# ZhangT-tech/MoCA-Video

Hardware: AMD Instinct MI355X
Metric: denoising UNet-steps/sec @16x320x512 fp16 (higher is better)
Workload: dtype f16

## Files before the change

include/moca_hip.h:

```cpp
#ifndef MOCA_HIP_H
#define MOCA_HIP_H

#include <stdint.h>

#ifdef __cplusplus
extern "C" {
#endif

#define MOCA_OK            0
#define MOCA_E_BADARG     -1
#define MOCA_E_LAUNCH     -2
#define MOCA_E_NODEVICE   -3
#define MOCA_E_GRAPH      -4

#define MOCA_A_LINEAR   0
#define MOCA_A_CONV3X3  1
#define MOCA_A_TCONV3   2

#define MOCA_EP_GEGLU   1
#define MOCA_EP_OUT_F32 2
#define MOCA_FORCE_SMALL_TILE 4
#define MOCA_EP_COLSUM 16
#define MOCA_EP_LN     32
#define MOCA_EP_GELU    8
// ... 44 lines not shown
    float       tattn_scale;
    const void* prefetch;
    int32_t     up_phase;
    int32_t     reserved4_;
    const void* a2;
    int32_t     lda2;
    int32_t     k1;
    int32_t     gstat_cpg;
    int32_t     gstat_coff;
    int32_t     wgroup_rows;
    int32_t     wgroup_stride;
} moca_gemm_params;

int moca_gemm_f16(const moca_gemm_params* p, void* stream);
int moca_gemm_colsum_rows(const moca_gemm_params* p);
int moca_gemm_ln_ok(const moca_gemm_params* p);
int moca_gemm_rowsum_cols(const moca_gemm_params* p);
int moca_gemm_lnfold_ok(const moca_gemm_params* p);
int moca_gemm_tattn_ok(const moca_gemm_params* p);
int moca_gemm_wgroup_ok(const moca_gemm_params* p);
int moca_gemm_cat_ok(const moca_gemm_params* p);
#define MOCA_ROUTE_SMALL64   1
#define MOCA_ROUTE_SMALL128  2
#define MOCA_ROUTE_GLDS128   3
#define MOCA_ROUTE_GLDS160   4
#define MOCA_ROUTE_G4        5
#define MOCA_ROUTE_W80       6
#define MOCA_ROUTE_W80W      7
#define MOCA_ROUTE_SQ256     8
#define MOCA_ROUTE_G4P       9
#define MOCA_ROUTE_SQP       10
#define MOCA_ROUTE_TATTN     11
#define MOCA_ROUTE_WS        12
int moca_gemm_route(const moca_gemm_params* p);
int moca_gemm_splitk_groupnorm_ok(const moca_gemm_params* p, int32_t HW, int32_t frames_per_stat);
int moca_gemm_splitk_groupnorm_f16(const moca_gemm_params* p, void* y, const float* gamma, const float* beta, int32_t HW,
                                   int32_t frames_per_stat, float eps, int32_t silu, int32_t write_x, void* stream);
int64_t moca_gemm_splitk_ws_bytes(int32_t M, int32_t N, int32_t splits);

int moca_groupnorm_nhwc_f16(const void* x, void* y, const float* gamma, const float* beta,
                            int32_t F, int32_t HW, int32_t C, int32_t frames_per_stat,
                            float eps, int32_t silu, float* ws, void* stream);
int64_t moca_groupnorm_ws_bytes(int32_t F, int32_t HW, int32_t C);
int moca_groupnorm_colsum_f16(const void* x, void* y, const float* gamma, const float* beta, const float* colsum,
                              int32_t tile_rows, int32_t F, int32_t HW, int32_t C, int32_t frames_per_stat,
                              float eps, int32_t silu, float* ws, void* stream);

int moca_groupnorm_fold_weights_f16(const void* w, const float* bias, const float* gamma, const float* beta, const int64_t* gstat,
                                    void* wg, float* bg, int32_t n_sg, int32_t N, int32_t K, int32_t ldw, int64_t count, float eps,
                                    void* stream);

int moca_groupnorm_gstat_f16(const void* x, void* y, const float* gamma, const float* beta, const int64_t* gstat,
                             int32_t F, int32_t HW, int32_t C, int32_t frames_per_stat,
                             float eps, int32_t silu, void* stream);
int moca_concat_channels_gstat_f16(const void* a, const void* b, void* out, int32_t F, int32_t HW, int32_t C1, int32_t C2,
                                   int32_t frames_per_stat, int64_t* gstat, void* stream);
int moca_groupnorm_gstat_cat_f16(const void* a, const void* b, void* y, const float* gamma, const float* beta,
                                 const int64_t* gstat_cat, const int64_t* gstat_b, int32_t Fb, int32_t F, int32_t HW, int32_t C1,
                                 int32_t C2, int32_t frames_per_stat, float eps, int32_t silu, void* stream);
int moca_gstat_accum_f16(const void* x, int32_t F, int32_t HW, int32_t C, int32_t frames_per_stat, int32_t cpg, int32_t coff,
                         int64_t* gstat, void* stream);
int moca_memset_zero(void* ptr, int64_t bytes, void* stream);

int moca_layernorm_f16(const void* x, void* y, const float* gamma, const float* beta,
                       int32_t M, int32_t C, float eps, void* stream);

// ... 117 lines not shown
int moca_base_ddim_step_f32(moca_fifo_state* state, float* x, const float* eps_c, const float* eps_u, const float* noise,
                            float* pred_x0, const float* coef, int32_t S, float cfg_scale, int32_t use_scale, int64_t n, void* stream);
int moca_mask_frame_sums_f32(const float* mask, float* sums, int32_t frames, int32_t HW, void* stream);

int moca_freq_mix_3d_f32(const float* x, const float* noise, const float* lpf, float* out,
                         int32_t C, int32_t T, int32_t H, int32_t W, float* ws, void* stream);
int64_t moca_freq_mix_ws_bytes(int32_t C, int32_t T, int32_t H, int32_t W);
int moca_freq_filter_f32(float* lpf, int32_t T, int32_t H, int32_t W, int32_t type, int32_t n,
                         double d_s, double d_t, void* stream);

int moca_graph_begin(void* stream);
int moca_graph_end(void* stream, void** graph_exec_out);
int moca_graph_launch(void* graph_exec, void* stream);
int moca_graph_destroy(void* graph_exec);
int moca_stream_create(void** stream_out);
int moca_stream_destroy(void* stream);
int moca_stream_sync(void* stream);
int moca_event_create(void** ev_out);
int moca_event_record(void* ev, void* stream);
int moca_event_elapsed_ms(void* ev_start, void* ev_stop, float* ms_out);
int moca_event_destroy(void* ev);

#define MOCA_TUNE_GEMM_W80   0
#define MOCA_TUNE_GEMM_G4    1
#define MOCA_TUNE_GEMM_SQ256 2
#define MOCA_TUNE_GEMM_WIDE  3
#define MOCA_TUNE_GN_SLAB    4
#define MOCA_TUNE_GEMM_G4P   5
#define MOCA_TUNE_GEMM_MF32  6
#define MOCA_TUNE_GEMM_SQP   7
#define MOCA_TUNE_SQP_WALK   8
#define MOCA_TUNE_SLAB_F16   9
#define MOCA_TUNE_GEMM_WS    10
#define MOCA_TUNE_COUNT      11
int moca_set_tuning(int32_t knob, int32_t value);
int moca_debug_clock_sampler(void* buf, int32_t blocks, int32_t nsamples, const int32_t* stop, void* stream);

int moca_device_info(char* name, int32_t len, int32_t* cu_count);
const char* moca_version(void);

#ifdef __cplusplus
}
#endif
#endif
```

moca_video_amd/csrc/gemm.hip:

```cpp
#include "gemm_launch.h"

namespace {

template <int BN, int AMODE>
__global__ __launch_bounds__(256, 2) void gemm_f16_kernel(const moca_gemm_params p) {
    constexpr int NT = BN / 64;
    constexpr int B_SLOTS = BN / 32;
    constexpr int A_BYTES = BM * ROW_BYTES;
    constexpr int B_BYTES = BN * ROW_BYTES;

    extern __shared__ __attribute__((aligned(16))) char smem[];
    char* sA = smem;
    char* sB = smem + 2 * A_BYTES;

    const int tid = threadIdx.x, lane = tid & 63, wave = tid >> 6;
    const int wave_m = wave >> 1, wave_n = wave & 1;

    const int tiles_m = (p.M + BM - 1) / BM;
    const int tiles_n = p.N / BN;
    const int nblk = tiles_m * tiles_n * p.splits;
    int logical;
    remap_block<BN>(nblk, logical);
    const int split = logical % p.splits;
    const int tile = logical / p.splits;
// ... 389 lines not shown
            const int c0 = ccol[i] - g * cpg;
            half8v r;
#pragma unroll
            for (int j = 0; j < 8; ++j) {
                float a = (float)v[i][j] * s_sc[c0 + j] + s_sh[c0 + j];
                if (silu) a = moca_silu(a);
                r[j] = (half_t)a;
            }
            *reinterpret_cast<half8v*>(y + (int64_t)mrow[i] * N + ccol[i]) = r;
        }
}

template <int BN, int AMODE>
int launch_gemm(const moca_gemm_params& p, hipStream_t st) {
    const int tiles_m = (p.M + BM - 1) / BM, tiles_n = p.N / BN;
    const int nblk = tiles_m * tiles_n * p.splits;
    constexpr int lds_pipe = 2 * (BM + BN) * ROW_BYTES;
    constexpr int lds_epi = BM * BN * 4;
    constexpr int lds = lds_pipe > lds_epi ? lds_pipe : lds_epi;
    if (!dyn_lds_once<&gemm_f16_kernel<BN, AMODE>>(lds)) return MOCA_E_LAUNCH;
    hipLaunchKernelGGL((gemm_f16_kernel<BN, AMODE>), dim3(nblk), dim3(256), lds, st, p);
    MOCA_CHECK_LAUNCH();
    return MOCA_OK;
}
int launch_gemm_small(int bn, const moca_gemm_params& p, hipStream_t st) {
    if (bn == 128) return with_gather(p, [&](auto am, auto) { return launch_gemm<128, decltype(am)::value>(p, st); });
    return with_gather(p, [&](auto am, auto) { return launch_gemm<64, decltype(am)::value>(p, st); });
}

enum Route : int {
    R_NONE = 0,
    R_SMALL64 = MOCA_ROUTE_SMALL64, R_SMALL128 = MOCA_ROUTE_SMALL128, R_GLDS128 = MOCA_ROUTE_GLDS128, R_GLDS160 = MOCA_ROUTE_GLDS160,
    R_G4 = MOCA_ROUTE_G4, R_W80 = MOCA_ROUTE_W80, R_W80W = MOCA_ROUTE_W80W, R_SQ256 = MOCA_ROUTE_SQ256, R_G4P = MOCA_ROUTE_G4P,
    R_SQP = MOCA_ROUTE_SQP, R_TATTN = MOCA_ROUTE_TATTN, R_WS = MOCA_ROUTE_WS,
};

void normalise_splits(moca_gemm_params& p) {
    if (p.splits < 1) p.splits = 1;
    if (p.splits > (p.K + BK - 1) / BK) p.splits = (p.K + BK - 1) / BK;
    if (p.splits > 1) {
        const int nkt = (p.K + BK - 1) / BK, kts = (nkt + p.splits - 1) / p.splits;
        p.splits = (nkt + kts - 1) / kts;
    }
}

inline int64_t a_span_bytes(const moca_gemm_params& p) {
    if (p.a_mode == MOCA_A_LINEAR) return ((int64_t)p.M * p.lda + 64) * 2;
    if (p.a_mode == MOCA_A_CONV3X3) return ((int64_t)(p.M / (p.outH * p.outW)) * p.inH * p.inW * p.C + 64) * 2;
    return ((int64_t)p.M * p.C + 64) * 2;
}
inline bool buffer_addressable(const moca_gemm_params& p) {
    if (p.a2 && ((int64_t)p.M * p.lda2 + 64) * 2 >= (1ll << 31)) return false;
    return a_span_bytes(p) < (1ll << 31) && (int64_t)p.N * p.ldw * 2 < (1ll << 31);
}

bool persistent_ok(const moca_gemm_params& p, int BN, int blocks) {
    if (p.a_mode != MOCA_A_LINEAR || p.splits != 1 || p.N % BN || p.K % 64 || !buffer_addressable(p)) return false;
    if (p.flags & ~(MOCA_EP_GEGLU | MOCA_EP_LNFOLD)) return false;
    if ((p.flags & MOCA_EP_GEGLU) && (p.residual || p.rowadd)) return false;
    return ((p.M + 255) / 256) * (p.N / BN) >= blocks;
}

Route route_of(const moca_gemm_params& p) {
    if (p.flags & MOCA_EP_TATTN) return R_TATTN;
    const int ws_mode = moca_tuning_get(MOCA_TUNE_GEMM_WS);
    if (ws_mode && moca_gemm_ws_ok(p) && (ws_mode == 2 || p.residual || p.M >= (1 << 17))) return R_WS;
    if (!p.a2 && p.wgroup_rows <= 0) {
        const int sqp_mode = moca_tuning_get(MOCA_TUNE_GEMM_SQP), g4p_mode = moca_tuning_get(MOCA_TUNE_GEMM_G4P);
        if (sqp_mode && persistent_ok(p, 256, SQP_BLOCKS) && (sqp_mode == 2 || (p.flags & MOCA_EP_GEGLU))) return R_SQP;
        if (g4p_mode && persistent_ok(p, 128, G4P_BLOCKS) && (g4p_mode == 2 || (p.flags & MOCA_EP_GEGLU))) return R_G4P;
    }
    const int w80_mode = moca_tuning_get(MOCA_TUNE_GEMM_W80);
    const int tiles320 = ((p.M + 319) / 320) * (p.N / 160);
    if (w80_mode && p.N % 160 == 0 && !(p.flags & (MOCA_EP_GEGLU | MOCA_EP_OUT_F32 | MOCA_FORCE_SMALL_TILE)) && p.M > 160 &&
        (tiles320 * p.splits >= 200 || w80_mode == 2) && fast_gather(p) && buffer_addressable(p)) {
        if (p.flags & MOCA_EP_LN) return R_W80W;
        const int wide_mode = moca_tuning_get(MOCA_TUNE_GEMM_WIDE);
        if (wide_mode == 0 || p.N % 320) return R_W80;
        return (p.a_mode == MOCA_A_LINEAR || wide_mode == 2) ? R_W80W : R_W80;
    }
    const int g4_mode = moca_tuning_get(MOCA_TUNE_GEMM_G4);
    const bool use_g4 = !(p.flags & MOCA_EP_OUT_F32) &&
                        (g4_mode == 2 || (g4_mode == 1 && (p.flags & MOCA_EP_GEGLU) && p.K <= 640 && p.M < (1 << 17)));
    const int sq256_mode = moca_tuning_get(MOCA_TUNE_GEMM_SQ256);
    if (sq256_mode && p.a_mode == MOCA_A_LINEAR && p.N % 256 == 0 && p.N >= 2560 && p.M >= 512 && fast_gather(p) && buffer_addressable(p) &&
        !(p.flags & (MOCA_EP_OUT_F32 | MOCA_FORCE_SMALL_TILE)) && ((p.M + 255) / 256) * (p.N / 256) * p.splits >= 200 &&
        (sq256_mode == 2 || !use_g4)) return R_SQ256;
    const int big_bn = (p.N % 128 == 0) ? 128 : (p.N % 160 == 0 ? 160 : 0);
    if (big_bn != 0 && p.M > 128 && !(p.flags & MOCA_FORCE_SMALL_TILE)) {
        if (big_bn == 128) return use_g4 ? R_G4 : R_GLDS128;
        return R_GLDS160;
    }
    return p.N % 128 == 0 ? R_SMALL128 : R_SMALL64;
}

constexpr int CAN_SPLITK = 1 << 16, CAN_A2 = 1 << 17, CAN_WGROUP = 1 << 18, CAN_UP_PHASE = 1 << 19;
constexpr int EP_STATS = MOCA_EP_COLSUM | MOCA_EP_GSTAT;
struct RouteInfo { int tm, tn, can; };
RouteInfo route_info(Route r) {
    constexpr int GLDS = MOCA_EP_GEGLU | MOCA_EP_OUT_F32 | EP_STATS | MOCA_EP_ROWSUM | MOCA_EP_LNFOLD | CAN_SPLITK | CAN_UP_PHASE;
    constexpr int W80 = EP_STATS | MOCA_EP_ROWSUM | MOCA_EP_LNFOLD | CAN_SPLITK | CAN_UP_PHASE | CAN_A2 | CAN_WGROUP;
    switch (r) {
        case R_SMALL64: return {BM, 64, MOCA_EP_OUT_F32 | MOCA_EP_GELU | CAN_SPLITK};
        case R_SMALL128: return {BM, 128, MOCA_EP_GEGLU | MOCA_EP_OUT_F32 | MOCA_EP_GELU | CAN_SPLITK};
        case R_GLDS128: return {256, 128, GLDS};
        case R_GLDS160: return {256, 160, GLDS};
        case R_G4: return {256, 128, MOCA_EP_GEGLU | MOCA_EP_LNFOLD | CAN_SPLITK | CAN_UP_PHASE};
        case R_W80: return {320, 160, W80};
        case R_W80W: return {160, 320, W80 | MOCA_EP_LN};
        case R_SQ256: return {256, 256, MOCA_EP_GEGLU | MOCA_EP_LNFOLD | CAN_SPLITK};
        case R_G4P: return {256, 128, MOCA_EP_GEGLU | MOCA_EP_LNFOLD};
        case R_SQP: return {256, 256, MOCA_EP_GEGLU | MOCA_EP_LNFOLD};
        case R_TATTN: return {320, 192, MOCA_EP_TATTN | MOCA_EP_LNFOLD};
        case R_WS: return {32, 80, MOCA_EP_ROWSUM | MOCA_EP_GSTAT | CAN_WGROUP};
        case R_NONE: break;
    }
    return {0, 0, 0};
}

bool route_can(Route r, const moca_gemm_params& p) {
    const RouteInfo ri = route_info(r);
    const int f = p.flags & ~(MOCA_FORCE_SMALL_TILE | MOCA_EP_SLABS);
    const int wants = f | (p.splits > 1 ? CAN_SPLITK : 0) | (p.a2 ? CAN_A2 : 0) | (p.wgroup_rows ? CAN_WGROUP : 0) | (p.up_phase ? CAN_UP_PHASE : 0);
    if (r == R_NONE || (wants & ~ri.can) || p.wgroup_rows < 0) return false;
    if (r == R_WS) return true;
    const bool linear1 = p.a_mode == MOCA_A_LINEAR && p.splits == 1;
    if (r == R_TATTN) {
        if (!linear1 || !fast_gather(p) || !buffer_addressable(p) || p.residual || p.rowadd || (p.flags & MOCA_FORCE_SMALL_TILE)) return false;
        if (p.N % 192 || p.T != 16 || p.HW <= 0 || p.HW % 20 || p.M % (16 * p.HW)) return false;
        if (p.ldo % 4 || p.ldo < p.N / 3) return false;
        return p.tattn_causal == 0 || (p.tattn_causal == 1 && p.tattn_scale > 0.f);
    }
    if ((f & EP_STATS) && (p.splits != 1 || (f & (MOCA_EP_GEGLU | MOCA_EP_OUT_F32)))) return false;
    if ((f & MOCA_EP_ROWSUM) && (p.splits != 1 || (f & (MOCA_EP_GEGLU | MOCA_EP_OUT_F32 | EP_STATS | MOCA_EP_LN | MOCA_EP_GELU)))) return false;
    if ((f & MOCA_EP_LN) && !(linear1 && p.N == 320 && !(f & EP_STATS))) return false;
    if ((f & MOCA_EP_LNFOLD) && !(linear1 && !(f & (MOCA_EP_OUT_F32 | EP_STATS | MOCA_EP_LN | MOCA_EP_ROWSUM | MOCA_EP_GELU)) &&
                                  !((r == R_GLDS128 || r == R_GLDS160) && (f & MOCA_EP_GEGLU)))) return false;
    if ((f & MOCA_EP_GELU) && (f & MOCA_EP_GEGLU)) return false;
    if (p.a2) {
        if (!linear1 || (f & ~(EP_STATS | MOCA_EP_ROWSUM))) return false;
        if (p.k1 <= 0 || p.k1 >= p.K || p.k1 % 64 || (p.K - p.k1) % 64 || p.lda % 8 || p.lda2 % 8 || p.lda < p.k1 || p.lda2 < p.K - p.k1) return false;
    }
    if (p.wgroup_rows) {
        if (!linear1 || p.a2 || p.wgroup_stride < p.N * p.ldw || (f & ~(EP_STATS | MOCA_EP_ROWSUM | MOCA_EP_LN))) return false;
        if (p.M % p.wgroup_rows || p.wgroup_rows % ri.tm) return false;
        if ((int64_t)(p.M / p.wgroup_rows) * p.wgroup_stride * 2 >= (1ll << 31)) return false;
    }
    if (p.up_phase && (p.splits != 1 || p.M <= 160 || !fast_gather(p) || p.residual || p.rowadd || (f & ~MOCA_EP_GSTAT) ||
                       (p.N % 128 && p.N % 160))) return false;
    return true;
}

Route checked_route(const moca_gemm_params& p) {
    const Route r = route_of(p);
    return route_can(r, p) ? r : R_NONE;
}

Route query_route(const moca_gemm_params* pp, int flag, moca_gemm_params& p) {
// ... 44 lines not shown
            if (p.up && (p.stride != 1 || p.outH != 2 * p.inH || p.outW != 2 * p.inW)) return R_NONE;
            if (!p.up && p.stride == 1 && (p.outH != p.inH || p.outW != p.inW)) return R_NONE;
            if (p.stride == 2 && (p.outH != (p.inH - 1) / 2 + 1 || p.outW != (p.inW - 1) / 2 + 1)) return R_NONE;
            if (p.M % (p.outH * p.outW)) return R_NONE;
            break;
        case MOCA_A_TCONV3:
            if (p.C % 8 || p.K != 3 * p.C || p.T <= 0 || p.HW <= 0 || p.M % (p.T * p.HW)) return R_NONE;
            break;
        default:
            return R_NONE;
    }
    if (p.a2 && p.a_mode != MOCA_A_LINEAR) return R_NONE;
    if (p.gstat_cpg < 0 || p.gstat_coff < 0 || ((p.gstat_cpg || p.gstat_coff) && !(p.flags & MOCA_EP_GSTAT))) return R_NONE;
    if (p.tattn_causal && !(p.flags & MOCA_EP_TATTN)) return R_NONE;
    const Route r = checked_route(p);
    if (r == R_NONE) return R_NONE;
    if ((p.flags & MOCA_EP_COLSUM) && !p.colsum) return R_NONE;
    if ((p.flags & MOCA_EP_LN) && !(p.ln_gamma && p.ln_beta && p.ln_out && p.ld_ln % 8 == 0)) return R_NONE;
    if ((p.flags & MOCA_EP_ROWSUM) && !p.rowsum) return R_NONE;
    if ((p.flags & MOCA_EP_LNFOLD) && !(p.lnf_part && p.lnf_wsum && p.lnf_nparts >= 1)) return R_NONE;
    if ((p.flags & MOCA_EP_GSTAT) &&
        !(p.gstat && !(p.flags & MOCA_EP_COLSUM) && p.gstat_rows > 0 && p.gstat_rows % route_info(r).tm == 0 && p.M % p.gstat_rows == 0 &&
          (p.gstat_cpg > 0 ? (p.gstat_coff + p.N - 1) / p.gstat_cpg < 32 : (p.N % 32 == 0 && p.gstat_coff == 0)))) return R_NONE;
    p.reserved4_ = 0;
    if ((int64_t)p.M * (geglu ? p.N / 2 : p.N) * 2 >= (128ll << 20)) p.reserved4_ |= 1;
    if (slab_f16(r, p)) p.reserved4_ |= 4;
    return r;
}

int launch_route(Route r, const moca_gemm_params& p, hipStream_t st) {
    switch (r) {
        case R_TATTN: return moca_gemm_w80s_launch(3, p, st);
        case R_WS: return moca_gemm_ws_launch(p, st);
        case R_SQP: return moca_gemm_sqp_launch(p, st);
        case R_G4P: return moca_gemm_g4p_launch(p, st);
        case R_W80: return moca_gemm_w80s_launch(0, p, st);
        case R_W80W: return moca_gemm_w80s_launch(1, p, st);
        case R_SQ256: return moca_gemm_w80s_launch(2, p, st);
        case R_G4: return moca_gemm_g4_launch(p, st);
        case R_GLDS128: return moca_gemm_glds_launch(128, p, st);
        case R_GLDS160: return moca_gemm_glds_launch(160, p, st);
        case R_SMALL128: return launch_gemm_small(128, p, st);
        case R_SMALL64: return launch_gemm_small(64, p, st);
        case R_NONE: break;
    }
    return MOCA_E_BADARG;
}

}

#ifdef MOCA_STAMPS
extern "C" int moca_debug_stamps(unsigned long long* host_out, int n_blocks) {
    if (n_blocks > STAMP_BLOCKS) n_blocks = STAMP_BLOCKS;
    return hipMemcpyFromSymbol(host_out, HIP_SYMBOL(g_stamps), (size_t)n_blocks * STAMP_SLOTS * 8) == hipSuccess ? 0 : -2;
}
#endif

extern "C" int moca_gemm_route(const moca_gemm_params* pp) {
    moca_gemm_params p;
    return prepare(pp, p);
}

extern "C" int moca_gemm_colsum_rows(const moca_gemm_params* pp) {
    moca_gemm_params p;
    return route_info(query_route(pp, (pp && (pp->flags & MOCA_EP_GSTAT)) ? 0 : MOCA_EP_COLSUM, p)).tm;
}
// ... 82 lines not shown
```

moca_video_amd/csrc/gemm_device.h:

```cpp
#ifndef MOCA_GEMM_DEVICE_H
#define MOCA_GEMM_DEVICE_H
#include "common.h"

namespace {

template <int V> struct int_c { static constexpr int value = V; };
struct yes_t { static constexpr bool value = true; };
struct no_t { static constexpr bool value = false; };

constexpr int BM = 128;
constexpr int BK = 64;
constexpr int MOCA_A_LINEAR2 = 3;
constexpr int ROW_BYTES = BK * 2;

struct Geo {
    int C, inH, inW, outH, outW, stride, up, T, HW;
};

__device__ __forceinline__ void remap_tile_2d(int tiles_m, int tiles_n, int xn, int& tile_m, int& tile_n) {
    const int xm = 8 / xn;
    const int sm = tiles_m / xm, sn = tiles_n / xn;
    const int b = blockIdx.x;
    const int xcd = b & 7, j = b >> 3;
    const int xi = xcd / xn, xj = xcd - xi * xn;
// ... 146 lines not shown
        } else if (AMODE == MOCA_A_CONV3X3) {
            const int ky = p.up_phase ? t >> 1 : t / 3, kx = p.up_phase ? t & 1 : t - ky * 3;
            const int limH = p.up ? 2 * p.inH : p.inH, limW = p.up ? 2 * p.inW : p.inW;
#pragma unroll
            for (int g = 0; g < NAP; ++g) {
                int iy = row_y[g] + ky, ix = row_x[g] + kx;
                const bool ok = t < (p.up_phase ? 4 : 9) && row_ok[g] && iy >= 0 && iy < limH && ix >= 0 && ix < limW;
                if (p.up) { iy >>= 1; ix >>= 1; }
                a_off[g] = ok ? (unsigned)(((row_off[g] + (int64_t)iy * p.inW + ix) * p.C + lch * 8) * 2) : OOB_OFF;
            }
        } else {
#pragma unroll
            for (int g = 0; g < NAP; ++g) {
                const int tt = row_y[g] + t - 1;
                const bool ok = t < 3 && row_ok[g] && tt >= 0 && tt < p.T;
                a_off[g] = ok ? (unsigned)(((row_off[g] + (int64_t)(t - 1) * p.HW) * p.C + lch * 8) * 2) : OOB_OFF;
            }
        }
    }

    __device__ __forceinline__ void seek(int kt) {
        kt_next = kt;
        const int t = AMODE == MOCA_A_LINEAR2 ? (kt >= tiles_per_tap ? 1 : 0) : kt / tiles_per_tap;
        tin = kt - t * tiles_per_tap;
        set_tap(t);
    }
    __device__ __forceinline__ void advance() {
        if (kt_next + 2 <= kt_last) {
            kt_next += 2;
            tin += 2;
            if (tin >= tiles_per_tap) { tin = 0; set_tap(tap + 1); }
        }
    }
    __device__ __forceinline__ unsigned a_soff() const { return (unsigned)(tin * KS * 2); }
    __device__ __forceinline__ unsigned w_soff() const { return (unsigned)(kt_next * KS * 2); }
};

__device__ __forceinline__ bool out_streams(const moca_gemm_params& p) { return p.reserved4_ & 1; }
__device__ __forceinline__ void st_out8(half_t* ptr, const half8v v, bool nt) {
#if defined(__HIP_DEVICE_COMPILE__)
    if (nt) asm volatile("global_store_dwordx4 %0, %1, off nt" :: "v"(ptr), "v"(v) : "memory");
    else *reinterpret_cast<half8v*>(ptr) = v;
#endif
}

template <bool NT>
__device__ __forceinline__ half8v ld_res8(const half_t* ptr) {
    if constexpr (NT) return __builtin_nontemporal_load(reinterpret_cast<const half8v*>(ptr));
    else return *reinterpret_cast<const half8v*>(ptr);
}

constexpr int EPI_U = 8;

template <int NTHREADS, bool NT>
__device__ __forceinline__ void store_fp16_tile_impl(const moca_gemm_params& p, const char* stage, int pitch, int rows, int out_bn,
                                                int m0, int on0, int tid) {
    const half_t* __restrict__ rowadd = reinterpret_cast<const half_t*>(p.rowadd);
    const half_t* __restrict__ resid = reinterpret_cast<const half_t*>(p.residual);
    constexpr bool nt_out = NT;
    const int chunks_per_row = out_bn / 8;
    const int total_chunks = rows * chunks_per_row;
    if (!rowadd && !resid) {
        const int upW = p.up_phase ? p.outW : 0, upC = p.up_phase ? 2 * p.outW * ((p.up_phase - 1) >> 1) + ((p.up_phase - 1) & 1) : 0;
        for (int idx = tid; idx < total_chunks; idx += NTHREADS) {
            const int row = idx / chunks_per_row, ch = idx - row * chunks_per_row;
            const int m = m0 + row;
// ... 326 lines not shown
```

moca_video_amd/csrc/gemm_diag.hip:

```cpp
#ifndef MOCA_DIAG_NAME
#error "gemm_diag.hip is the unit of the diagnostic builds: compile it with -DMOCA_DIAG_NAME"
#endif
#include "gemm.hip"
#include "gemm_tiled.hip"
#include "gemm_persistent.hip"
```

moca_video_amd/csrc/gemm_launch.h:

```cpp
#ifndef MOCA_GEMM_LAUNCH_H
#define MOCA_GEMM_LAUNCH_H
#include "gemm_device.h"

int moca_gemm_glds_launch(int bn, const moca_gemm_params& p, hipStream_t st);
int moca_gemm_g4_launch(const moca_gemm_params& p, hipStream_t st);
int moca_gemm_w80s_launch(int shape, const moca_gemm_params& p, hipStream_t st);
int moca_gemm_g4p_launch(const moca_gemm_params& p, hipStream_t st);
int moca_gemm_sqp_launch(const moca_gemm_params& p, hipStream_t st);

namespace {

constexpr int G4P_BLOCKS = 512;
constexpr int SQP_BLOCKS = 256;

static int choose_xcd_n(const moca_gemm_params& p, int tiles_m, int tiles_n, int BN) {
    if (p.splits != 1 || p.a_mode != MOCA_A_LINEAR) return 1;
    const double Wtot = (double)p.N * p.K * 2, Atot = (double)p.M * p.K * 2;
    auto cost = [&](int xn) {
        const int xm = 8 / xn;
        const double wsub = (double)(tiles_n / xn) * BN * p.K * 2;
        return (wsub <= 3.6e6 ? xm * Wtot : tiles_m * Wtot) + xn * Atot;
    };
    double best = cost(1);
    int best_xn = 1;
    for (int xn = 2; xn <= 8; xn *= 2) {
        if (tiles_m % (8 / xn) || tiles_n % xn) continue;
        const double c = cost(xn);
        if (c < 0.8 * best) { best = c; best_xn = xn; }
    }
    return best_xn;
}

inline bool fast_gather(const moca_gemm_params& p) {
    return (p.a_mode == MOCA_A_LINEAR) ? (p.K % BK == 0 && p.K <= 8192) : (p.C % BK == 0 && p.C <= 8192);
}
template <typename F>
int with_gather(const moca_gemm_params& p, F f) {
    const bool fast = fast_gather(p);
    if (p.a_mode == MOCA_A_LINEAR) return fast ? f(int_c<MOCA_A_LINEAR>{}, yes_t{}) : f(int_c<MOCA_A_LINEAR>{}, no_t{});
    if (p.a_mode == MOCA_A_CONV3X3) return fast ? f(int_c<MOCA_A_CONV3X3>{}, yes_t{}) : f(int_c<MOCA_A_CONV3X3>{}, no_t{});
    return fast ? f(int_c<MOCA_A_TCONV3>{}, yes_t{}) : f(int_c<MOCA_A_TCONV3>{}, no_t{});
// ... 16 lines not shown
```

moca_video_amd/csrc/runtime.hip:

```cpp
#include "common.h"
#include <string.h>
#include <stdio.h>
#include <stdlib.h>

extern "C" int moca_graph_begin(void* stream) {
    if (hipStreamBeginCapture(moca_stream(stream), hipStreamCaptureModeThreadLocal) != hipSuccess) return MOCA_E_GRAPH;
    return MOCA_OK;
}

extern "C" int moca_graph_end(void* stream, void** graph_exec_out) {
    if (!graph_exec_out) return MOCA_E_BADARG;
    hipGraph_t g = nullptr;
    if (hipStreamEndCapture(moca_stream(stream), &g) != hipSuccess || !g) return MOCA_E_GRAPH;
    hipGraphExec_t ge = nullptr;
    hipError_t e = hipGraphInstantiate(&ge, g, nullptr, nullptr, 0);
    (void)hipGraphDestroy(g);
    if (e != hipSuccess || !ge) return MOCA_E_GRAPH;
    *graph_exec_out = reinterpret_cast<void*>(ge);
    return MOCA_OK;
}

extern "C" int moca_graph_launch(void* graph_exec, void* stream) {
    if (!graph_exec) return MOCA_E_BADARG;
    if (hipGraphLaunch(reinterpret_cast<hipGraphExec_t>(graph_exec), moca_stream(stream)) != hipSuccess) return MOCA_E_GRAPH;
// ... 65 lines not shown
    const int64_t n16 = bytes / 16;
    int blocks = (int)((n16 + 255) / 256);
    if (blocks < 1) blocks = 1;
    if (blocks > 1024) blocks = 1024;
    hipLaunchKernelGGL(zero_kernel, dim3(blocks), dim3(256), 0, moca_stream(stream), reinterpret_cast<uint4*>(ptr), n16,
                       reinterpret_cast<unsigned char*>(ptr) + n16 * 16, (int)(bytes - n16 * 16));
    MOCA_CHECK_LAUNCH();
    return MOCA_OK;
}

__global__ __launch_bounds__(64) void clock_sampler_kernel(unsigned long long* __restrict__ buf, int nsamples, const volatile int* stop) {
#if defined(__HIP_DEVICE_COMPILE__)
    if (threadIdx.x) return;
    unsigned long long* b = buf + (size_t)blockIdx.x * nsamples * 2;
    for (int i = 0; i < nsamples; ++i) {
        unsigned long long t, r;
        asm volatile("s_memtime %0\n\ts_memrealtime %1\n\ts_waitcnt lgkmcnt(0)" : "=s"(t), "=s"(r)::"memory");
        b[2 * i] = t;
        b[2 * i + 1] = r;
        if (stop && *stop) break;
        __builtin_amdgcn_s_sleep(127);
        __builtin_amdgcn_s_sleep(127);
    }
#endif
}
extern "C" int moca_debug_clock_sampler(void* buf, int32_t blocks, int32_t nsamples, const int32_t* stop, void* stream) {
    if (!buf || blocks < 1 || blocks > 64 || nsamples < 1 || nsamples > (1 << 20)) return MOCA_E_BADARG;
    hipLaunchKernelGGL(clock_sampler_kernel, dim3(blocks), dim3(64), 0, moca_stream(stream), reinterpret_cast<unsigned long long*>(buf), nsamples,
                       reinterpret_cast<const volatile int*>(stop));
    MOCA_CHECK_LAUNCH();
    return MOCA_OK;
}

static int g_tuning[MOCA_TUNE_COUNT] = {1, 1, 1, 1, 1, 1, 0, 1, 0, 0, 1};
int moca_tuning_get(int knob) { return (knob >= 0 && knob < MOCA_TUNE_COUNT) ? g_tuning[knob] : 0; }
extern "C" int moca_set_tuning(int32_t knob, int32_t value) {
    if (knob < 0 || knob >= MOCA_TUNE_COUNT || value < 0 || value > 2) return MOCA_E_BADARG;
    const int old = g_tuning[knob];
    g_tuning[knob] = value;
    return old;
}
```

moca_video_amd/lib.py:

```python
from __future__ import annotations

import ctypes as C
import os

import torch

_HERE = os.path.dirname(os.path.abspath(__file__))
LIB_PATH = os.environ.get("MOCA_HIP_LIB") or os.path.join(_HERE, "libmoca_hip.so")

MOCA_A_LINEAR, MOCA_A_CONV3X3, MOCA_A_TCONV3 = 0, 1, 2
MOCA_EP_GEGLU, MOCA_EP_OUT_F32, MOCA_FORCE_SMALL_TILE, MOCA_EP_GELU, MOCA_EP_COLSUM, MOCA_EP_LN = 1, 2, 4, 8, 16, 32
MOCA_EP_ROWSUM, MOCA_EP_LNFOLD, MOCA_EP_GSTAT, MOCA_EP_TATTN, MOCA_EP_SLABS = 64, 128, 256, 512, 1024
MOCA_TUNE_GEMM_W80, MOCA_TUNE_GEMM_G4, MOCA_TUNE_GEMM_SQ256, MOCA_TUNE_GEMM_WIDE, MOCA_TUNE_GN_SLAB, MOCA_TUNE_GEMM_G4P, MOCA_TUNE_GEMM_MF32, MOCA_TUNE_GEMM_SQP, MOCA_TUNE_SQP_WALK = 0, 1, 2, 3, 4, 5, 6, 7, 8
MOCA_TUNE_SLAB_F16 = 9
MOCA_TUNE_GEMM_WS = 10
(MOCA_ROUTE_SMALL64, MOCA_ROUTE_SMALL128, MOCA_ROUTE_GLDS128, MOCA_ROUTE_GLDS160, MOCA_ROUTE_G4, MOCA_ROUTE_W80, MOCA_ROUTE_W80W,
 MOCA_ROUTE_SQ256, MOCA_ROUTE_G4P, MOCA_ROUTE_SQP, MOCA_ROUTE_TATTN, MOCA_ROUTE_WS) = range(1, 13)

_ERR = {0: "ok", -1: "bad argument (shape/alignment contract)", -2: "HIP launch/runtime error",
        -3: "no gfx950 device", -4: "graph capture/replay failed"}


class MocaHipError(RuntimeError):
    pass


class GemmParams(C.Structure):
    _fields_ = [
        ("a", C.c_void_p), ("w", C.c_void_p), ("out", C.c_void_p), ("bias", C.c_void_p),
        ("rowadd", C.c_void_p), ("residual", C.c_void_p), ("splitk_ws", C.c_void_p),
        ("M", C.c_int32), ("N", C.c_int32), ("K", C.c_int32),
        ("lda", C.c_int32), ("ldw", C.c_int32), ("ldo", C.c_int32), ("ldr", C.c_int32), ("ld_rowadd", C.c_int32),
        ("rowadd_div", C.c_int32), ("a_mode", C.c_int32), ("C", C.c_int32),
        ("inH", C.c_int32), ("inW", C.c_int32), ("outH", C.c_int32), ("outW", C.c_int32),
        ("stride", C.c_int32), ("up", C.c_int32), ("T", C.c_int32), ("HW", C.c_int32),
        ("flags", C.c_int32), ("splits", C.c_int32), ("nopad_lo", C.c_int32), ("prefetch_kib", C.c_int32),
        ("tattn_causal", C.c_int32),
        ("colsum", C.c_void_p), ("ln_gamma", C.c_void_p), ("ln_beta", C.c_void_p), ("ln_out", C.c_void_p),
        ("ld_ln", C.c_int32), ("ln_eps", C.c_float),
        ("rowsum", C.c_void_p), ("lnf_part", C.c_void_p), ("lnf_wsum", C.c_void_p),
        ("lnf_nparts", C.c_int32), ("reserved2_", C.c_int32),
        ("gstat", C.c_void_p), ("gstat_rows", C.c_int32), ("tattn_scale", C.c_float),
        ("prefetch", C.c_void_p), ("up_phase", C.c_int32), ("reserved4_", C.c_int32),
        ("a2", C.c_void_p), ("lda2", C.c_int32), ("k1", C.c_int32), ("gstat_cpg", C.c_int32), ("gstat_coff", C.c_int32),
        ("wgroup_rows", C.c_int32), ("wgroup_stride", C.c_int32),
    ]


class FifoState(C.Structure):
    _fields_ = [("head", C.c_int32), ("iter", C.c_int32), ("seed_lo", C.c_uint32), ("seed_hi", C.c_uint32),
# ... 152 lines not shown
```

Measured before the change: 61.76.

## Add intra-block split-K GEMM route for mid-sized deep-K linears

Adds a new GEMM kernel where eight waves in a block each take a slice of K for an 80x80 output tile, then reduce their partials through LDS before applying bias and residual. It is routed by default for linear and tconv GEMMs with K>=1024 and 128-256 tiles. The aim is to fill the CUs on GEMMs whose output has too few tiles to occupy the device, without a global split-K workspace. The cost is an LDS reduction step and a per-wave pipeline only two stages deep, which may be less efficient than the existing routes.

```diff
diff --git a/include/moca_hip.h b/include/moca_hip.h
--- a/include/moca_hip.h
+++ b/include/moca_hip.h
@@ -100,6 +100,7 @@
 #define MOCA_ROUTE_SQP       10
 #define MOCA_ROUTE_TATTN     11
 #define MOCA_ROUTE_WS        12
+#define MOCA_ROUTE_KS        13
 int moca_gemm_route(const moca_gemm_params* p);
 int moca_gemm_splitk_groupnorm_ok(const moca_gemm_params* p, int32_t HW, int32_t frames_per_stat);
 int moca_gemm_splitk_groupnorm_f16(const moca_gemm_params* p, void* y, const float* gamma, const float* beta, int32_t HW,
@@ -283,7 +284,8 @@
 #define MOCA_TUNE_SQP_WALK   8
 #define MOCA_TUNE_SLAB_F16   9
 #define MOCA_TUNE_GEMM_WS    10
-#define MOCA_TUNE_COUNT      11
+#define MOCA_TUNE_GEMM_KS    11
+#define MOCA_TUNE_COUNT      12
 int moca_set_tuning(int32_t knob, int32_t value);
 int moca_debug_clock_sampler(void* buf, int32_t blocks, int32_t nsamples, const int32_t* stop, void* stream);
 
diff --git a/moca_video_amd/csrc/gemm.hip b/moca_video_amd/csrc/gemm.hip
--- a/moca_video_amd/csrc/gemm.hip
+++ b/moca_video_amd/csrc/gemm.hip
@@ -445,7 +445,7 @@
     R_NONE = 0,
     R_SMALL64 = MOCA_ROUTE_SMALL64, R_SMALL128 = MOCA_ROUTE_SMALL128, R_GLDS128 = MOCA_ROUTE_GLDS128, R_GLDS160 = MOCA_ROUTE_GLDS160,
     R_G4 = MOCA_ROUTE_G4, R_W80 = MOCA_ROUTE_W80, R_W80W = MOCA_ROUTE_W80W, R_SQ256 = MOCA_ROUTE_SQ256, R_G4P = MOCA_ROUTE_G4P,
-    R_SQP = MOCA_ROUTE_SQP, R_TATTN = MOCA_ROUTE_TATTN, R_WS = MOCA_ROUTE_WS,
+    R_SQP = MOCA_ROUTE_SQP, R_TATTN = MOCA_ROUTE_TATTN, R_WS = MOCA_ROUTE_WS, R_KS = MOCA_ROUTE_KS,
 };
 
 void normalise_splits(moca_gemm_params& p) {
@@ -474,10 +474,21 @@
     return ((p.M + 255) / 256) * (p.N / BN) >= blocks;
 }
 
+bool ks_ok(const moca_gemm_params& p) {
+    if (p.a_mode != MOCA_A_LINEAR && p.a_mode != MOCA_A_TCONV3) return false;
+    if (p.splits != 1 || p.flags || p.a2 || p.wgroup_rows || p.rowadd || p.up_phase) return false;
+    return p.N % 80 == 0 && p.K % 64 == 0 && fast_gather(p) && buffer_addressable(p);
+}
+
 Route route_of(const moca_gemm_params& p) {
     if (p.flags & MOCA_EP_TATTN) return R_TATTN;
     const int ws_mode = moca_tuning_get(MOCA_TUNE_GEMM_WS);
     if (ws_mode && moca_gemm_ws_ok(p) && (ws_mode == 2 || p.residual || p.M >= (1 << 17))) return R_WS;
+    const int ks_mode = moca_tuning_get(MOCA_TUNE_GEMM_KS);
+    if (ks_mode && ks_ok(p)) {
+        const int tiles80 = ((p.M + 79) / 80) * (p.N / 80);
+        if (ks_mode == 2 || (p.K >= 1024 && tiles80 >= 128 && tiles80 <= 256)) return R_KS;
+    }
     if (!p.a2 && p.wgroup_rows <= 0) {
         const int sqp_mode = moca_tuning_get(MOCA_TUNE_GEMM_SQP), g4p_mode = moca_tuning_get(MOCA_TUNE_GEMM_G4P);
         if (sqp_mode && persistent_ok(p, 256, SQP_BLOCKS) && (sqp_mode == 2 || (p.flags & MOCA_EP_GEGLU))) return R_SQP;
@@ -526,6 +537,7 @@
         case R_SQP: return {256, 256, MOCA_EP_GEGLU | MOCA_EP_LNFOLD};
         case R_TATTN: return {320, 192, MOCA_EP_TATTN | MOCA_EP_LNFOLD};
         case R_WS: return {32, 80, MOCA_EP_ROWSUM | MOCA_EP_GSTAT | CAN_WGROUP};
+        case R_KS: return {80, 80, 0};
         case R_NONE: break;
     }
     return {0, 0, 0};
@@ -537,6 +549,7 @@
     const int wants = f | (p.splits > 1 ? CAN_SPLITK : 0) | (p.a2 ? CAN_A2 : 0) | (p.wgroup_rows ? CAN_WGROUP : 0) | (p.up_phase ? CAN_UP_PHASE : 0);
     if (r == R_NONE || (wants & ~ri.can) || p.wgroup_rows < 0) return false;
     if (r == R_WS) return true;
+    if (r == R_KS) return ks_ok(p);
     const bool linear1 = p.a_mode == MOCA_A_LINEAR && p.splits == 1;
     if (r == R_TATTN) {
         if (!linear1 || !fast_gather(p) || !buffer_addressable(p) || p.residual || p.rowadd || (p.flags & MOCA_FORCE_SMALL_TILE)) return false;
@@ -647,6 +660,7 @@
     switch (r) {
         case R_TATTN: return moca_gemm_w80s_launch(3, p, st);
         case R_WS: return moca_gemm_ws_launch(p, st);
+        case R_KS: return moca_gemm_ks_launch(p, st);
         case R_SQP: return moca_gemm_sqp_launch(p, st);
         case R_G4P: return moca_gemm_g4p_launch(p, st);
         case R_W80: return moca_gemm_w80s_launch(0, p, st);
diff --git a/moca_video_amd/csrc/gemm_device.h b/moca_video_amd/csrc/gemm_device.h
--- a/moca_video_amd/csrc/gemm_device.h
+++ b/moca_video_amd/csrc/gemm_device.h
@@ -202,6 +202,10 @@
             if (tin >= tiles_per_tap) { tin = 0; set_tap(tap + 1); }
         }
     }
+    __device__ __forceinline__ void step() {
+        ++kt_next;
+        if (++tin >= tiles_per_tap) { tin = 0; set_tap(tap + 1); }
+    }
     __device__ __forceinline__ unsigned a_soff() const { return (unsigned)(tin * KS * 2); }
     __device__ __forceinline__ unsigned w_soff() const { return (unsigned)(kt_next * KS * 2); }
 };
diff --git a/moca_video_amd/csrc/gemm_diag.hip b/moca_video_amd/csrc/gemm_diag.hip
--- a/moca_video_amd/csrc/gemm_diag.hip
+++ b/moca_video_amd/csrc/gemm_diag.hip
@@ -4,3 +4,4 @@
 #include "gemm.hip"
 #include "gemm_tiled.hip"
 #include "gemm_persistent.hip"
+#include "gemm_ks.hip"
diff --git a/moca_video_amd/csrc/gemm_ks.hip b/moca_video_amd/csrc/gemm_ks.hip
--- /dev/null
+++ b/moca_video_amd/csrc/gemm_ks.hip
@@ -0,0 +1,208 @@
+#include "gemm_launch.h"
+
+namespace {
+
+constexpr int KS_T = 80;
+constexpr int KS_STAGE = 2 * KS_T * 128;
+constexpr int KS_LDS = 8 * KS_STAGE;
+constexpr int KS_HALF = 40;
+constexpr int KS_PITCH = 84;
+constexpr int KS_PART = KS_HALF * KS_PITCH;
+static_assert(8 * KS_PART * 4 <= KS_LDS, "the eight half partials fit into the ring memory");
+
+template <int AMODE, bool RES>
+__global__ __launch_bounds__(512, 2) void gemm_ks_kernel(const moca_gemm_params p) {
+#if defined(__HIP_DEVICE_COMPILE__)
+    constexpr int MT = 5, NT = 5, KD = 64, RB = 128;
+    constexpr int NAP = 5;
+
+    extern __shared__ __attribute__((aligned(16))) char smem[];
+
+    const int tid = threadIdx.x, lane = tid & 63;
+    const int wave = __builtin_amdgcn_readfirstlane(tid >> 6);
+
+    const int tiles_m = (p.M + KS_T - 1) / KS_T;
+    const int tiles_n = p.N / KS_T;
+    const int nblk = tiles_m * tiles_n;
+    if (prefetch_block(p, nblk, 512)) return;
+    int tile_m, tile_n;
+    const int xcd_n = p.reserved4_ >> 8;
+    if (xcd_n > 1) {
+        remap_tile_2d(tiles_m, tiles_n, xcd_n, tile_m, tile_n);
+    } else {
+        int logical;
+        remap_block<KS_T>(nblk, logical);
+        tile_m = logical / tiles_n; tile_n = logical % tiles_n;
+    }
+    const int m0 = tile_m * KS_T, n0 = tile_n * KS_T;
+
+    const int nk = p.K / KD;
+    const int kt_begin = nk * wave / 8, kt_end = nk * (wave + 1) / 8;
+    const int n = kt_end - kt_begin;
+
+    const int lrow = lane >> 3, pch = lane & 7;
+    const int lch0 = pch ^ (lrow >> 1), lch1 = pch ^ ((lrow >> 1) | 4);
+    BGather<AMODE, NAP, KD> ga0(p, lch0, kt_begin, kt_end - 1), ga1(p, lch1, kt_begin, kt_end - 1);
+#pragma unroll
+    for (int g = 0; g < NAP; ++g) {
+        ga0.init_row(g, m0 + g * 16 + lrow);
+        ga1.init_row(g, m0 + g * 16 + 8 + lrow);
+    }
+    const unsigned w_off0 = (unsigned)(((int64_t)(n0 + lrow) * p.ldw + lch0 * 8) * 2);
+    const unsigned w_off1 = (unsigned)(((int64_t)(n0 + 8 + lrow) * p.ldw + lch1 * 8) * 2);
+    const unsigned w_pair = (unsigned)p.ldw * 32u;
+    const __amdgpu_buffer_rsrc_t rsrc_a = __builtin_amdgcn_make_buffer_rsrc(const_cast<void*>(p.a), 0, OOB_OFF, 0x00020000);
+    const __amdgpu_buffer_rsrc_t rsrc_w = __builtin_amdgcn_make_buffer_rsrc(const_cast<void*>(p.w), 0, OOB_OFF, 0x00020000);
+
+    const lds_ptr stage = (lds_ptr)smem + wave * KS_STAGE;
+    auto issue_tile = [&]() {
+        const unsigned a_s = ga0.a_soff(), w_s = ga0.w_soff();
+#pragma unroll
+        for (int g = 0; g < NAP; ++g) {
+            __builtin_amdgcn_raw_ptr_buffer_load_lds(rsrc_a, stage + (2 * g) * 1024, 16, ga0.a_off[g], a_s, 0, 0);
+            __builtin_amdgcn_raw_ptr_buffer_load_lds(rsrc_a, stage + (2 * g + 1) * 1024, 16, ga1.a_off[g], a_s, 0, 0);
+        }
+#pragma unroll
+        for (int g = 0; g < NAP; ++g) {
+            __builtin_amdgcn_raw_ptr_buffer_load_lds(rsrc_w, stage + KS_T * RB + (2 * g) * 1024, 16, w_off0, w_s + g * w_pair, 0, 0);
+            __builtin_amdgcn_raw_ptr_buffer_load_lds(rsrc_w, stage + KS_T * RB + (2 * g + 1) * 1024, 16, w_off1, w_s + g * w_pair, 0, 0);
+        }
+    };
+
+    const int fr = lane & 15, fg = lane >> 4;
+    f32x4 acc[MT][NT];
+#pragma unroll
+    for (int mt = 0; mt < MT; ++mt)
+#pragma unroll
+        for (int nt = 0; nt < NT; ++nt) acc[mt][nt] = f32x4{0.f, 0.f, 0.f, 0.f};
+
+    const int f_row = wave * KS_STAGE + fr * RB;
+    const int f_off[2] = {f_row + ((fg ^ ((fr >> 1) & 7)) << 4), f_row + (((4 + fg) ^ ((fr >> 1) & 7)) << 4)};
+    half8v af[2][MT], bf[2][NT];
+    auto read_tile = [&]() {
+#pragma unroll
+        for (int s = 0; s < 2; ++s) {
+#pragma unroll
+            for (int r = 0; r < NT; ++r) bf[s][r] = *reinterpret_cast<const half8v*>(smem + f_off[s] + KS_T * RB + r * 16 * RB);
+#pragma unroll
+            for (int r = 0; r < MT; ++r) af[s][r] = *reinterpret_cast<const half8v*>(smem + f_off[s] + r * 16 * RB);
+        }
+    };
+    auto mfma_tile = [&]() {
+        __builtin_amdgcn_s_setprio(1);
+#pragma unroll
+        for (int s = 0; s < 2; ++s)
+#pragma unroll
+            for (int mt = 0; mt < MT; ++mt)
+#pragma unroll
+                for (int nt = 0; nt < NT; ++nt)
+                    acc[mt][nt] = __builtin_amdgcn_mfma_f32_16x16x32_f16(bf[s][nt], af[s][mt], acc[mt][nt], 0, 0, 0);
+        __builtin_amdgcn_s_setprio(0);
+    };
+
+    if (n > 0) {
+        ga0.seek(kt_begin);
+        ga1.seek(kt_begin);
+        issue_tile();
+    }
+    for (int i = 0; i + 1 < n; ++i) {
+        asm volatile("s_waitcnt vmcnt(0)" ::: "memory");
+        __builtin_amdgcn_sched_barrier(0);
+        read_tile();
+        asm volatile("s_waitcnt lgkmcnt(0)" ::: "memory");
+        __builtin_amdgcn_sched_barrier(0);
+        ga0.step();
+        ga1.step();
+        issue_tile();
+        __builtin_amdgcn_sched_barrier(0);
+        mfma_tile();
+        __builtin_amdgcn_sched_barrier(0);
+    }
+    if (n > 0) {
+        asm volatile("s_waitcnt vmcnt(0)" ::: "memory");
+        __builtin_amdgcn_sched_barrier(0);
+        read_tile();
+        asm volatile("s_waitcnt lgkmcnt(0)" ::: "memory");
+        __builtin_amdgcn_sched_barrier(0);
+        mfma_tile();
+        __builtin_amdgcn_sched_barrier(0);
+    }
+    asm volatile("s_waitcnt vmcnt(0) lgkmcnt(0)" ::: "memory");
+    __syncthreads();
+
+    float* part = reinterpret_cast<float*>(smem);
+    const half_t* __restrict__ resid = reinterpret_cast<const half_t*>(p.residual);
+    half_t* outp = reinterpret_cast<half_t*>(p.out);
+    const bool nt_out = out_streams(p);
+    const int srow = wave * 5 + lane / 10, c8 = (lane % 10) * 8;
+    const bool sum_lane = lane < 50;
+#pragma unroll
+    for (int h = 0; h < 2; ++h) {
+#pragma unroll
+        for (int mt = 0; mt < MT; ++mt) {
+            const int lr = mt * 16 + fr - h * KS_HALF;
+            if (lr >= 0 && lr < KS_HALF) {
+#pragma unroll
+                for (int nt = 0; nt < NT; ++nt)
+                    *reinterpret_cast<f32x4*>(part + wave * KS_PART + lr * KS_PITCH + nt * 16 + 4 * fg) = acc[mt][nt];
+            }
+        }
+        __syncthreads();
+        const int m = m0 + h * KS_HALF + srow;
+        if (sum_lane && m < p.M) {
+            const float* src = part + srow * KS_PITCH + c8;
+            f32x4 s0 = *reinterpret_cast<const f32x4*>(src), s1 = *reinterpret_cast<const f32x4*>(src + 4);
+#pragma unroll
+            for (int q = 1; q < 8; ++q) {
+                s0 += *reinterpret_cast<const f32x4*>(src + q * KS_PART);
+                s1 += *reinterpret_cast<const f32x4*>(src + q * KS_PART + 4);
+            }
+            if (p.bias) {
+                s0 += *reinterpret_cast<const f32x4*>(p.bias + n0 + c8);
+                s1 += *reinterpret_cast<const f32x4*>(p.bias + n0 + c8 + 4);
+            }
+            if constexpr (RES) {
+                const half8v e = *reinterpret_cast<const half8v*>(resid + (int64_t)m * p.ldr + n0 + c8);
+#pragma unroll
+                for (int j = 0; j < 4; ++j) { s0[j] += (float)e[j]; s1[j] += (float)e[4 + j]; }
+            }
+            half8v o;
+#pragma unroll
+            for (int j = 0; j < 4; ++j) { o[j] = (half_t)s0[j]; o[4 + j] = (half_t)s1[j]; }
+            st_out8(outp + (int64_t)m * p.ldo + n0 + c8, o, nt_out);
+        }
+        if (h == 0) __syncthreads();
+    }
+#endif
+}
+
+int ks_xcd_n(int tiles_m, int tiles_n) {
+    int best = 1, best_rows = 0;
+    for (int xn = 1; xn <= 8; xn *= 2) {
+        const int xm = 8 / xn;
+        if (tiles_m % xm || tiles_n % xn) continue;
+        const int rows = tiles_m / xm + tiles_n / xn;
+        if (best_rows == 0 || rows < best_rows) { best = xn; best_rows = rows; }
+    }
+    return best_rows ? best : 1;
+}
+
+template <int AMODE, bool RES>
+int launch_gemm_ks(const moca_gemm_params& p, hipStream_t st) {
+    const int tiles_m = (p.M + KS_T - 1) / KS_T, tiles_n = p.N / KS_T;
+    const int nblk = tiles_m * tiles_n;
+    moca_gemm_params pl = p;
+    pl.reserved4_ = (pl.reserved4_ & 0xff) | (ks_xcd_n(tiles_m, tiles_n) << 8);
+    if (!dyn_lds_once<&gemm_ks_kernel<AMODE, RES>>(KS_LDS)) return MOCA_E_LAUNCH;
+    hipLaunchKernelGGL((gemm_ks_kernel<AMODE, RES>), dim3(nblk + prefetch_blocks(pl)), dim3(512), KS_LDS, st, pl);
+    MOCA_CHECK_LAUNCH();
+    return MOCA_OK;
+}
+
+}
+
+int moca_gemm_ks_launch(const moca_gemm_params& p, hipStream_t st) {
+    if (p.a_mode != MOCA_A_LINEAR && p.a_mode != MOCA_A_TCONV3) return MOCA_E_BADARG;
+    if (p.a_mode == MOCA_A_LINEAR) return p.residual ? launch_gemm_ks<MOCA_A_LINEAR, true>(p, st) : launch_gemm_ks<MOCA_A_LINEAR, false>(p, st);
+    return p.residual ? launch_gemm_ks<MOCA_A_TCONV3, true>(p, st) : launch_gemm_ks<MOCA_A_TCONV3, false>(p, st);
+}
diff --git a/moca_video_amd/csrc/gemm_launch.h b/moca_video_amd/csrc/gemm_launch.h
--- a/moca_video_amd/csrc/gemm_launch.h
+++ b/moca_video_amd/csrc/gemm_launch.h
@@ -7,6 +7,7 @@
 int moca_gemm_w80s_launch(int shape, const moca_gemm_params& p, hipStream_t st);
 int moca_gemm_g4p_launch(const moca_gemm_params& p, hipStream_t st);
 int moca_gemm_sqp_launch(const moca_gemm_params& p, hipStream_t st);
+int moca_gemm_ks_launch(const moca_gemm_params& p, hipStream_t st);
 
 namespace {
 
diff --git a/moca_video_amd/csrc/runtime.hip b/moca_video_amd/csrc/runtime.hip
--- a/moca_video_amd/csrc/runtime.hip
+++ b/moca_video_amd/csrc/runtime.hip
@@ -121,7 +121,7 @@
     return MOCA_OK;
 }
 
-static int g_tuning[MOCA_TUNE_COUNT] = {1, 1, 1, 1, 1, 1, 0, 1, 0, 0, 1};
+static int g_tuning[MOCA_TUNE_COUNT] = {1, 1, 1, 1, 1, 1, 0, 1, 0, 0, 1, 1};
 int moca_tuning_get(int knob) { return (knob >= 0 && knob < MOCA_TUNE_COUNT) ? g_tuning[knob] : 0; }
 extern "C" int moca_set_tuning(int32_t knob, int32_t value) {
     if (knob < 0 || knob >= MOCA_TUNE_COUNT || value < 0 || value > 2) return MOCA_E_BADARG;
diff --git a/moca_video_amd/lib.py b/moca_video_amd/lib.py
--- a/moca_video_amd/lib.py
+++ b/moca_video_amd/lib.py
@@ -14,8 +14,9 @@
 MOCA_TUNE_GEMM_W80, MOCA_TUNE_GEMM_G4, MOCA_TUNE_GEMM_SQ256, MOCA_TUNE_GEMM_WIDE, MOCA_TUNE_GN_SLAB, MOCA_TUNE_GEMM_G4P, MOCA_TUNE_GEMM_MF32, MOCA_TUNE_GEMM_SQP, MOCA_TUNE_SQP_WALK = 0, 1, 2, 3, 4, 5, 6, 7, 8
 MOCA_TUNE_SLAB_F16 = 9
 MOCA_TUNE_GEMM_WS = 10
+MOCA_TUNE_GEMM_KS = 11
 (MOCA_ROUTE_SMALL64, MOCA_ROUTE_SMALL128, MOCA_ROUTE_GLDS128, MOCA_ROUTE_GLDS160, MOCA_ROUTE_G4, MOCA_ROUTE_W80, MOCA_ROUTE_W80W,
- MOCA_ROUTE_SQ256, MOCA_ROUTE_G4P, MOCA_ROUTE_SQP, MOCA_ROUTE_TATTN, MOCA_ROUTE_WS) = range(1, 13)
+ MOCA_ROUTE_SQ256, MOCA_ROUTE_G4P, MOCA_ROUTE_SQP, MOCA_ROUTE_TATTN, MOCA_ROUTE_WS, MOCA_ROUTE_KS) = range(1, 14)
 
 _ERR = {0: "ok", -1: "bad argument (shape/alignment contract)", -2: "HIP launch/runtime error",
         -3: "no gfx950 device", -4: "graph capture/replay failed"}
```

Measured after the change: 61.73. Within noise of the previous version (-0.0%).
